# colinsongf/keyword_spotting

Measured on AMD Instinct MI355X. Metric: mel-frames/s (real-time 10 ms-hop audio streams sustained = value/100), higher is better.
Workload: dtype f32

## Files before the change

keyword_spotting_amd/csrc/gru_resident.hip:

```cpp
#include <cstddef>

#include "gru_device.h"
#include "launch.h"
#include "window_device.h"

namespace kws {

#if KWS_RESIDENT_VGPR_FORM
template <class... A> __device__ __forceinline__ void resident_prefence(A&...) {}
template <class... A> __device__ __forceinline__ void resident_fence(A&...) { __builtin_amdgcn_sched_barrier(0); }
#else
template <class... A> __device__ __forceinline__ void resident_prefence(A&... a) { mfma_prefence(a...); }
template <class... A> __device__ __forceinline__ void resident_fence(A&... a) { mfma_fence(a...); }
#endif


#if KWS_RESIDENT_VGPR_FORM
constexpr int resident_kreg(int kcx, bool first, bool last, bool window) { return first ? kcx : (last && window) ? 10 : 16; }
#else
constexpr int resident_kreg(int, bool first, bool, bool) { return first ? 0 : 2; }
#endif
constexpr size_t resident_lds_bytes(int kcx, bool first, bool last, bool window) {
    size_t n = 2 * 8 * 64 * 16 + (size_t)4 * (kcx - resident_kreg(kcx, first, last, window)) * 64 * 16;
    if (!first) n += 8 * 64 * 16;
    if (last) n += kPartialRingLdsBytes;
    if (first) n += (size_t)64 * xs_stride(kcx) * 4;
    return n;
}

template <int KCX, bool FIRST, bool LAST, bool MASKED, bool WINDOW>
__device__ __forceinline__ void gru_layer_resident_body(const GruLayerParams& p) {
    static_assert(!WINDOW || (LAST && !FIRST), "the window tail belongs to the last layer of a stack");
    static_assert(!WINDOW || !MASKED, "the window tail refuses seq_len");
    constexpr int H = 128, NT = 8, KCH = 32;
    const int tid = threadIdx.x;
    const int w = __builtin_amdgcn_readfirstlane(tid >> 6);
    const int lane = tid & 63, g = lane >> 4, s = lane & 15;
    const int n_groups = (p.B + kStreamsPerGroup - 1) / kStreamsPerGroup;
    int group = blockIdx.x;
    int b_raw = group * kStreamsPerGroup + s;
    bool bvalid = b_raw < p.B;
    int b = bvalid ? b_raw : p.B - 1;
    const int T = p.T;
    const int n0 = 2 * w, n1 = 2 * w + 1;

    extern __shared__ __attribute__((aligned(16))) char smem[];
    f32x4* hbuf = reinterpret_cast<f32x4*>(smem);
    f32x4* rhbuf = hbuf + NT * 64;
    constexpr int KREG = resident_kreg(KCX, FIRST, LAST, WINDOW), KL = KCX - KREG;
    static_assert(KREG >= 0 && KREG <= KCX && 192 + 4 * KREG <= 256, "the register chunks share the 256 AGPRs with the recurrent weights");
    f32x4* wlds = rhbuf + NT * 64;
    f32x4* xsb = wlds + 4 * KL * 64;
    char* const lds_tail = reinterpret_cast<char*>(xsb + (FIRST ? 0 : NT * 64));
    static_assert(resident_lds_bytes(KCX, FIRST, LAST, WINDOW) + (WINDOW ? kWinTailWordsBytes : 0) <= 160 * 1024, "LDS per CU");
    float* const pring = reinterpret_cast<float*>(lds_tail);
    int8_t* const cwords = WINDOW ? reinterpret_cast<int8_t*>(lds_tail + kPartialRingLdsBytes) : nullptr;
    const uint8_t* win_dl = reinterpret_cast<const uint8_t*>(cwords) + 16 * kWinTailWordsStride;
    constexpr size_t kWinOffset = offsetof(GruLayerParams, win);
    if constexpr (WINDOW) window_tail_prepare(window_tail_params_from_kernarg(kWinOffset), const_cast<uint8_t*>(win_dl), tid);
    constexpr int kXsStride = xs_stride(KCX);
    float* xs = reinterpret_cast<float*>(lds_tail + (LAST ? kPartialRingLdsBytes : 0));

    float wgh[2][2][KCH];
    float wch[2][KCH];
    float wcx[2][KCX];
    float wgx[KREG ? KREG : 1][4];
    const f32x4* wh4 = reinterpret_cast<const f32x4*>(p.wh);
#pragma unroll
    for (int j = 0; j < 2; ++j) {
        const int n = 2 * w + j;
#pragma unroll
        for (int k4 = 0; k4 < KCH / 4; ++k4) {
            const f32x4 vr = wh4[((n * 3 + 0) * (KCH / 4) + k4) * 64 + lane];
            const f32x4 vu = wh4[((n * 3 + 1) * (KCH / 4) + k4) * 64 + lane];
            const f32x4 vc = wh4[((n * 3 + 2) * (KCH / 4) + k4) * 64 + lane];
#pragma unroll
            for (int e = 0; e < 4; ++e) {
                wgh[j][0][4 * k4 + e] = vr[e];
                wgh[j][1][4 * k4 + e] = vu[e];
                wch[j][4 * k4 + e] = vc[e];
            }
        }
    }
    if constexpr (FIRST) {
#pragma unroll
        for (int j = 0; j < 2; ++j)
#pragma unroll
            for (int kc = 0; kc < KCX; ++kc) wcx[j][kc] = p.wx[(((2 * w + j) * 3 + 2) * KCX + kc) * 64 + lane];
#pragma unroll
        for (int kc = 0; kc < KCX; ++kc) {
            f32x4 v;
            v.x = p.wx[((n0 * 3 + 0) * KCX + kc) * 64 + lane];
            v.y = p.wx[((n0 * 3 + 1) * KCX + kc) * 64 + lane];
            v.z = p.wx[((n1 * 3 + 0) * KCX + kc) * 64 + lane];
            v.w = p.wx[((n1 * 3 + 1) * KCX + kc) * 64 + lane];
            if (kc < KREG) { const int kr = kc < KREG ? kc : 0; wgx[kr][0] = v[0]; wgx[kr][1] = v[1]; wgx[kr][2] = v[2]; wgx[kr][3] = v[3]; }
            else wlds[(w * KL + kc - KREG) * 64 + lane] = v;
        }
    } else {
        const f32x4* wx4 = reinterpret_cast<const f32x4*>(p.wx);
#pragma unroll
        for (int j = 0; j < 2; ++j)
#pragma unroll
            for (int k4 = 0; k4 < KCX / 4; ++k4) {
                const f32x4 vc = wx4[(((2 * w + j) * 3 + 2) * (KCX / 4) + k4) * 64 + lane];
#pragma unroll
                for (int e = 0; e < 4; ++e) wcx[j][4 * k4 + e] = vc[e];
            }
#pragma unroll
        for (int k4 = 0; k4 < KCX / 4; ++k4) {
            const f32x4 r0 = wx4[((n0 * 3 + 0) * (KCX / 4) + k4) * 64 + lane];
            const f32x4 u0 = wx4[((n0 * 3 + 1) * (KCX / 4) + k4) * 64 + lane];
            const f32x4 r1 = wx4[((n1 * 3 + 0) * (KCX / 4) + k4) * 64 + lane];
            const f32x4 u1 = wx4[((n1 * 3 + 1) * (KCX / 4) + k4) * 64 + lane];
#pragma unroll
            for (int e = 0; e < 4; ++e) {
                const f32x4 v = {r0[e], u0[e], r1[e], u1[e]};
                const int kc = 4 * k4 + e, kr = kc < KREG ? kc : 0;
                if (kc < KREG) { wgx[kr][0] = v[0]; wgx[kr][1] = v[1]; wgx[kr][2] = v[2]; wgx[kr][3] = v[3]; }
                else wlds[(w * KL + kc - KREG) * 64 + lane] = v;
            }
        }
    }
#pragma unroll
    for (int j = 0; j < 2; ++j) {
#pragma unroll
        for (int kc = 0; kc < KCH; ++kc) {
            asm volatile("" : "+a"(wgh[j][0][kc]));
            asm volatile("" : "+a"(wgh[j][1][kc]));
            asm volatile("" : "+a"(wch[j][kc]));
        }
    }
#if KWS_RESIDENT_VGPR_FORM
    if constexpr (KREG > 0) {
#pragma unroll
        for (int kc = 0; kc < KREG; ++kc)
#pragma unroll
            for (int e = 0; e < 4; ++e) asm volatile("" : "+a"(wgx[kc][e]));
    }
#endif
    asm volatile("s_nop 7" ::: "memory");
    f32x4 bias_r[2], bias_u[2], bias_c[2];
#pragma unroll
    for (int j = 0; j < 2; ++j) {
        const int n = 2 * w + j;
        bias_r[j] = ld4(p.bias + 0 * H + n * 16 + 4 * g);
        bias_u[j] = ld4(p.bias + 1 * H + n * 16 + 4 * g);
        bias_c[j] = ld4(p.bias + 2 * H + n * 16 + 4 * g);
    }
    float wfc[2][4];
    f32x4 bfc4 = splat4(0.f);
    if (LAST) {
#pragma unroll
        for (int j = 0; j < 2; ++j)
#pragma unroll
            for (int e = 0; e < 4; ++e) wfc[j][e] = p.wfc[((2 * w + j) * 4 + e) * 64 + lane];
        if (w == 0) bfc4 = ld4(p.bfc + 4 * g);
    }

    int len_s = T;
    int carry = -1;
    f32x4 hreg[2];
    const float4* xl_src = nullptr;
    const float4* xprev = nullptr;
    const float4* xg_next = nullptr;
    constexpr int XQ = KCX;
    const int xl_row = lane / XQ, xl_q = lane % XQ;
    const bool xl_active = FIRST && lane < 4 * XQ;
    auto enter_group = [&]() {
        b_raw = group * kStreamsPerGroup + s;
        bvalid = b_raw < p.B;
        b = bvalid ? b_raw : p.B - 1;
        const bool do_reset = p.reset != nullptr && p.reset[b] != 0;
        if constexpr (MASKED) len_s = p.seq_len ? p.seq_len[b] - p.t_base : T;
#pragma unroll
        for (int j = 0; j < 2; ++j) {
            const int n = 2 * w + j;
            hreg[j] = do_reset ? splat4(0.f) : ld4(p.state_in + (size_t)b * H + n * 16 + 4 * g);
            hbuf[n * 64 + lane] = hreg[j];
        }
        if (LAST) {
            carry = carried_word(p.prev_word, p.reset, group * kStreamsPerGroup + 4 * w + (lane >> 4), p.B);
        }
        if constexpr (FIRST) {
            const int xl_b = min(group * kStreamsPerGroup + 4 * w + (xl_active ? xl_row : 0), p.B - 1);
            xl_src = reinterpret_cast<const float4*>(p.x_mel + (size_t)xl_b * (p.t_stride ? p.t_stride : T) * p.I) + xl_q;
        } else {
            xprev = p.x_prev + (size_t)group * T * NT * 64 + lane;
            xg_next = xprev + ((size_t)(1 < T ? 1 : 0) * NT + n0) * 64;
        }
    };

    constexpr bool kIssueAtEnd = FIRST && !LAST;
    float4 xl_inflight = make_float4(0.f, 0.f, 0.f, 0.f);
    auto coop_issue = [&](int t_req) {
        const int t = t_req < T ? t_req : T - 1;
        if (xl_active) xl_inflight = xl_src[(size_t)t * XQ];
    };
    auto coop_commit = [&]() {
        if (xl_active) {
            float* dst = xs + (4 * (4 * w + xl_row)) * kXsStride + xl_q;
            dst[0 * kXsStride] = xl_inflight.x;
            dst[1 * kXsStride] = xl_inflight.y;
            dst[2 * kXsStride] = xl_inflight.z;
            dst[3 * kXsStride] = xl_inflight.w;
        }
    };
    float xbuf0[KCX];
    auto read_xs = [&](float (&dst)[KCX]) {
        const float* row = xs + (4 * s + g) * kXsStride;
#pragma unroll
        for (int k4 = 0; k4 < KCX / 4; ++k4) {
            const f32x4 v = *reinterpret_cast<const f32x4*>(row + 4 * k4);
            dst[4 * k4 + 0] = v[0]; dst[4 * k4 + 1] = v[1]; dst[4 * k4 + 2] = v[2]; dst[4 * k4 + 3] = v[3];
        }
        if constexpr (KCX % 4 >= 2) {
            const f32x2 v = *reinterpret_cast<const f32x2*>(row + (KCX / 4) * 4);
            dst[(KCX / 4) * 4 + 0] = v[0]; dst[(KCX / 4) * 4 + 1] = v[1];
        }
        if constexpr (KCX % 2 == 1) dst[KCX - 1] = row[KCX - 1];
    };
    auto load_x_slice = [&](float (&dst)[KCX], int t_req, const int sl) {
        if constexpr (!FIRST) {
            const int t = t_req < T ? t_req : T - 1;
            const float4 v = xprev[((size_t)t * NT + sl) * 64];
            dst[4 * sl + 0] = v.x; dst[4 * sl + 1] = v.y; dst[4 * sl + 2] = v.z; dst[4 * sl + 3] = v.w;
        }
    };
    float4 xg_inflight[2];
    auto group_issue = [&](int t_req) {
        if constexpr (!FIRST) {
            xg_inflight[0] = xg_next[0];
            xg_inflight[1] = xg_next[64];
            if (t_req + 1 < T) xg_next += NT * 64;
        }
    };
    auto group_commit = [&]() {
        if constexpr (!FIRST) {
#pragma unroll
            for (int j = 0; j < 2; ++j)
                xsb[(2 * w + j) * 64 + lane] = (f32x4){xg_inflight[j].x, xg_inflight[j].y, xg_inflight[j].z, xg_inflight[j].w};
        }
    };
    auto read_x_slice = [&](float (&dst)[KCX], const int sl) {
        if constexpr (!FIRST) {
            const f32x4 v = xsb[sl * 64 + lane];
            dst[4 * sl + 0] = v[0]; dst[4 * sl + 1] = v[1]; dst[4 * sl + 2] = v[2]; dst[4 * sl + 3] = v[3];
        }
    };

    f32x4 acc_r[2], acc_u[2], acc_c[2];
    auto gates_x_part = [&](const float (&xB)[KCX], auto k0_, auto k1_, auto pin_) {
        constexpr int K0 = decltype(k0_)::value, K1 = decltype(k1_)::value;
        constexpr bool PIN = decltype(pin_)::value;
        constexpr int R0 = K0 < KREG ? KREG : K0;
        f32x4 ring[3];
        if (R0 < K1) ring[R0 % 3] = wlds[(w * KL + R0 - KREG) * 64 + lane];
        if (R0 + 1 < K1) ring[(R0 + 1) % 3] = wlds[(w * KL + R0 + 1 - KREG) * 64 + lane];
#pragma unroll
        for (int kc = K0; kc < K1; ++kc) {
            if (kc + 2 < K1 && kc + 2 >= R0 + 2) ring[(kc + 2) % 3] = wlds[(w * KL + kc + 2 - KREG) * 64 + lane];
            if (PIN) __builtin_amdgcn_sched_barrier(0);
            const int kr = kc < KREG ? kc : 0;
            const f32x4 a4 = kc < KREG ? (f32x4){wgx[kr][0], wgx[kr][1], wgx[kr][2], wgx[kr][3]} : ring[kc % 3];
            acc_r[0] = mfma4(a4.x, xB[kc], acc_r[0]);
            acc_u[0] = mfma4(a4.y, xB[kc], acc_u[0]);
            acc_r[1] = mfma4(a4.z, xB[kc], acc_r[1]);
            acc_u[1] = mfma4(a4.w, xB[kc], acc_u[1]);
            if (PIN) __builtin_amdgcn_sched_barrier(0);
        }
    };
    using pinned = std::true_type;
    constexpr int KSPLIT = KCX / 2;
    using k_lo = std::integral_constant<int, 0>;
    using k_mid = std::integral_constant<int, KSPLIT>;
    using k_hi = std::integral_constant<int, KCX>;
    auto cand_x = [&](const float (&xB)[KCX]) {
#pragma unroll
        for (int j = 0; j < 2; ++j) acc_c[j] = bias_c[j];
#pragma unroll
        for (int kc = 0; kc < KCX; ++kc) {
            acc_c[0] = mfma4(wcx[0][kc], xB[kc], acc_c[0]);
            acc_c[1] = mfma4(wcx[1][kc], xB[kc], acc_c[1]);
        }
    };

    f32x4 hb_a, hb_b;

    auto frame = [&](int t, float (&xcur)[KCX], float (&xnxt)[KCX]) {
        resident_prefence(acc_r[0], acc_u[0], acc_r[1], acc_u[1]);
#pragma unroll
        for (int nn = 0; nn < NT; ++nn) {
            const f32x4 hb = (nn & 1) ? hb_b : hb_a;
            if (nn + 2 < NT) {
                if (nn & 1) hb_b = hbuf[(nn + 2) * 64 + lane]; else hb_a = hbuf[(nn + 2) * 64 + lane];
            }
            if constexpr (FIRST) { if (!kIssueAtEnd && nn == 0) coop_issue(t + 2); }
            else { if (nn == 0) group_issue(t + 2); read_x_slice(xnxt, nn); }
            __builtin_amdgcn_sched_barrier(0);
#pragma unroll
            for (int e = 0; e < 4; ++e) {
                const int kc = 4 * nn + e;
                const float hv = hb[e];
                KWS_MFMA_A(acc_r[0], wgh[0][0][kc], hv);
                KWS_MFMA_A(acc_u[0], wgh[0][1][kc], hv);
                KWS_MFMA_A(acc_r[1], wgh[1][0][kc], hv);
                KWS_MFMA_A(acc_u[1], wgh[1][1][kc], hv);
            }
        }
        resident_fence(acc_r[0], acc_u[0], acc_r[1], acc_u[1]);
        if constexpr (FIRST) read_xs(xcur);
        f32x4 u[2];
#pragma unroll
        for (int j = 0; j < 2; ++j) {
            const f32x2 r_lo = sigmoid2((f32x2){acc_r[j][0], acc_r[j][1]});
            const f32x2 r_hi = sigmoid2((f32x2){acc_r[j][2], acc_r[j][3]});
            const f32x2 rh_lo = r_lo * (f32x2){hreg[j][0], hreg[j][1]};
            const f32x2 rh_hi = r_hi * (f32x2){hreg[j][2], hreg[j][3]};
            rhbuf[(2 * w + j) * 64 + lane] = (f32x4){rh_lo.x, rh_lo.y, rh_hi.x, rh_hi.y};
        }
#pragma unroll
        for (int j = 0; j < 2; ++j) {
            const f32x2 u_lo = sigmoid2((f32x2){acc_u[j][0], acc_u[j][1]});
            const f32x2 u_hi = sigmoid2((f32x2){acc_u[j][2], acc_u[j][3]});
            u[j] = (f32x4){u_lo.x, u_lo.y, u_hi.x, u_hi.y};
        }
#pragma unroll
        for (int j = 0; j < 2; ++j) { acc_r[j] = bias_r[j]; acc_u[j] = bias_u[j]; }
        __builtin_amdgcn_sched_barrier(0);
        gates_x_part(xcur, k_lo{}, k_mid{}, pinned{});
        lds_barrier();
        hb_a = rhbuf[0 * 64 + lane];
        hb_b = rhbuf[1 * 64 + lane];
        group_commit();
        gates_x_part(xcur, k_mid{}, k_hi{}, pinned{});

        resident_prefence(acc_c[0], acc_c[1]);
#pragma unroll
        for (int nn = 0; nn < NT; ++nn) {
            const f32x4 rb = (nn & 1) ? hb_b : hb_a;
            if (nn + 2 < NT) {
                if (nn & 1) hb_b = rhbuf[(nn + 2) * 64 + lane]; else hb_a = rhbuf[(nn + 2) * 64 + lane];
            }
            __builtin_amdgcn_sched_barrier(0);
#pragma unroll
            for (int e = 0; e < 4; ++e) {
                const int kc = 4 * nn + e;
                const float rv = rb[e];
                KWS_MFMA_A(acc_c[0], wch[0][kc], rv);
                KWS_MFMA_A(acc_c[1], wch[1][kc], rv);
            }
        }
        resident_fence(acc_c[0], acc_c[1]);
        const unsigned live = !MASKED || t < len_s ? 0xffffffffu : 0u;
        f32x4 hout[2];
#pragma unroll
        for (int j = 0; j < 2; ++j) {
#pragma unroll
            for (int h2 = 0; h2 < 2; ++h2) {
                const f32x2 c = tanh2((f32x2){acc_c[j][2 * h2], acc_c[j][2 * h2 + 1]});
                const f32x2 uu = {u[j][2 * h2], u[j][2 * h2 + 1]};
                const f32x2 hh = {hreg[j][2 * h2], hreg[j][2 * h2 + 1]};
                const f32x2 hn = __builtin_elementwise_fma(uu, hh, (1.0f - uu) * c);
                if constexpr (!MASKED) {
                    hreg[j][2 * h2] = hn.x;
                    hreg[j][2 * h2 + 1] = hn.y;
                    continue;
                }
                hreg[j][2 * h2] = bitsel(live, hn.x, hh.x);
                hreg[j][2 * h2 + 1] = bitsel(live, hn.y, hh.y);
                if (LAST) {
                    hout[j][2 * h2] = bitsel(live, hn.x, 0.f);
                    hout[j][2 * h2 + 1] = bitsel(live, hn.y, 0.f);
                }
            }
        }
#pragma unroll
        for (int j = 0; j < 2; ++j) acc_c[j] = bias_c[j];
        constexpr int NCX = 2 * KCX;
        constexpr int NPOST = NCX >= 32 ? 16 : 8;
        constexpr int NPRE = NCX - NPOST;
        auto cand_x_mfma = [&](auto mc) {
            constexpr int m = decltype(mc)::value, kc = m / 2;
            if constexpr (m % 2 == 0) acc_c[0] = mfma4(wcx[0][kc], xcur[kc], acc_c[0]);
            else acc_c[1] = mfma4(wcx[1][kc], xcur[kc], acc_c[1]);
        };
        if constexpr (FIRST) {
            coop_commit();
            if constexpr (kIssueAtEnd) coop_issue(t + 3);
        }
#pragma unroll
        for (int j = 0; j < 2; ++j) {
            hbuf[(2 * w + j) * 64 + lane] = hreg[j];
            if (!LAST) {
                const f32x4 o = hreg[j];
                p.h_out[((size_t)group * T + t) * NT * 64 + (2 * w + j) * 64 + lane] =
                    make_float4(o[0], o[1], o[2], o[3]);
            }
        }
        if constexpr (LAST) {
            __builtin_amdgcn_sched_barrier(0);
            f32x4 accf = bfc4;
#pragma unroll
            for (int j = 0; j < 2; ++j)
#pragma unroll
                for (int e = 0; e < 4; ++e) accf = mfma4(wfc[j][e], MASKED ? hout[j][e] : hreg[j][e], accf);
            if (g < 2) *reinterpret_cast<f32x4*>(partial_slot(pring, t) + (w * 16 + s) * 8 + 4 * g) = accf;
        }
        __builtin_amdgcn_sched_barrier(0);
        static_for<0, NPRE>(cand_x_mfma);
        __builtin_amdgcn_sched_barrier(0);
        lds_barrier();
        hb_a = hbuf[0 * 64 + lane];
        hb_b = hbuf[1 * 64 + lane];
        __builtin_amdgcn_sched_barrier(0);
        static_for<NPRE, NCX>(cand_x_mfma);
        __builtin_amdgcn_sched_barrier(0);
        if constexpr (LAST) {
            if (((t + 1) & (kRingFrames - 1)) == 0 || t == T - 1) {
                const int t0 = t & ~(kRingFrames - 1);
                epilogue_flush_partials(p, pring, cwords, group, t0, t - t0 + 1, w, lane, t == T - 1, carry);
            }
        }
    };

    for (; group < n_groups; group += gridDim.x) {
    enter_group();
    if constexpr (!FIRST) {
        if (T > 0) {
            group_issue(1);
#pragma unroll
            for (int sl = 0; sl < NT; ++sl) load_x_slice(xbuf0, 0, sl);
            group_commit();
        }
    }
    __syncthreads();
    if (T > 0) {
        if constexpr (FIRST) {
            coop_issue(0);
            coop_commit();
            __syncthreads();
            read_xs(xbuf0);
            coop_issue(1);
        }
#pragma unroll
        for (int j = 0; j < 2; ++j) { acc_r[j] = bias_r[j]; acc_u[j] = bias_u[j]; }
        gates_x_part(xbuf0, k_lo{}, k_hi{}, pinned{});
        hb_a = hbuf[0 * 64 + lane];
        hb_b = hbuf[1 * 64 + lane];
        cand_x(xbuf0);
        if constexpr (FIRST) {
            __syncthreads();
            coop_commit();
            if constexpr (kIssueAtEnd) coop_issue(2);
            __syncthreads();
        }
    }
    for (int t = 0; t < T; ++t) frame(t, xbuf0, xbuf0);

    if (bvalid) {
#pragma unroll
        for (int j = 0; j < 2; ++j)
            *reinterpret_cast<f32x4*>(p.state_out + (size_t)b * H + (2 * w + j) * 16 + 4 * g) = hreg[j];
    }
    __syncthreads();
    if constexpr (WINDOW) {
        const WindowTail win = window_tail_params_from_kernarg(kWinOffset);
        WindowTailRegs<2> wreq;
        window_tail_request<2>(win, p.B, group * kStreamsPerGroup, tid, wreq);
        window_tail<2>(win, p.B, group * kStreamsPerGroup, T, cwords, kWinTailWordsStride, win_dl, reinterpret_cast<char*>(hbuf), tid, wreq);
        __syncthreads();
    }
    }
}

template <int KCX, bool FIRST, bool LAST, bool WINDOW = false>
__global__ void __launch_bounds__(256) __attribute__((amdgpu_waves_per_eu(1, 1)))
gru_layer_resident(const GruLayerParams p) { gru_layer_resident_body<KCX, FIRST, LAST, false, WINDOW>(p); }
template <int KCX, bool FIRST, bool LAST>
__global__ void __launch_bounds__(256) __attribute__((amdgpu_waves_per_eu(1, 1)))
gru_layer_resident_masked(const GruLayerParams p) { gru_layer_resident_body<KCX, FIRST, LAST, true, false>(p); }
template <int KCX, bool FIRST, bool LAST, bool MASKED>
inline constexpr auto resident_kernel = MASKED ? &gru_layer_resident_masked<KCX, FIRST, LAST> : &gru_layer_resident<KCX, FIRST, LAST, false>;

int gru_resident_kcx(int in_dim, bool first) { return first ? (in_dim + 3) / 4 : 32; }

bool gru_resident_supported(int hidden, int in_dim, bool first) {
    if (hidden != 128) return false;
    if (!first) return in_dim == 128;
    return in_dim == 32 || in_dim == 40 || in_dim == 48 || in_dim == 60 || in_dim == 64;
}

bool gru_resident_takes_window(bool first, bool last) { return last && !first; }

hipError_t launch_gru_layer_resident(const GruLayerParams& p, bool first, bool last, hipStream_t st) {
    const bool window = p.win.tab != nullptr;
    const size_t lds = resident_lds_bytes(p.KCX, first, last, window);
    const dim3 grid(persistent_grid(p.B));
    if (window) {
        if (!gru_resident_takes_window(first, last) || p.seq_len) return hipErrorInvalidValue;
        return launch_lds<gru_layer_resident<32, false, true, true>>(grid, dim3(256), lds + kWinTailWordsBytes, st, p);
    }
    return with_bool(p.seq_len != nullptr, [&](auto ma) {
        return with_bool(last, [&](auto la) {
            if (!first) return launch_lds<resident_kernel<32, false, la(), ma()>>(grid, dim3(256), lds, st, p);
            return with_int<8, 10, 12, 15, 16>(p.KCX, [&](auto kcx) {
                return launch_lds<resident_kernel<kcx(), true, la(), ma()>>(grid, dim3(256), lds, st, p);
            });
        });
    });
}

}
```

keyword_spotting_amd/csrc/kws_internal.h:

```cpp
#pragma once
#include <hip/hip_runtime.h>
#include <stdint.h>

#include "kws_amd.h"

#if defined(KWS_FAULT_INJECT) || defined(KWS_ABL_NOFLUSH) || defined(KWS_ABL_NOMEL) || defined(KWS_F16_TIMING) || defined(KWS_FE_TIMING) || \
    defined(KWS_FE_OCC) || defined(KWS_FE_FT) || defined(KWS_FE_SF) || defined(KWS_FE_NOSTAGE) || defined(KWS_FE_NODFT) || defined(KWS_FE_NOMEL) || \
    defined(KWS_OABL_NODIV) || defined(KWS_OABL_NODOT) || defined(KWS_OVERLAP_MIN_T) || defined(KWS_EXP_F16_WLO_ZERO)
#ifndef KWS_VARIANT_BUILD
#error "an experiment switch (KWS_FAULT_INJECT / KWS_ABL_* / KWS_*_TIMING / KWS_FE_* / KWS_OABL_* / KWS_OVERLAP_MIN_T) is defined in a product build: use tools/build_variant.sh"
#endif
#endif
#ifdef KWS_VARIANT_BUILD
#define KWS_VARIANT_TAG_1(name) "; " #name
#ifdef KWS_FAULT_INJECT
#define KWS_TAG_FAULT KWS_VARIANT_TAG_1(FAULT_INJECT)
#else
#define KWS_TAG_FAULT ""
#endif
#ifdef KWS_ABL_NOFLUSH
#define KWS_TAG_NOFLUSH KWS_VARIANT_TAG_1(ABL_NOFLUSH)
#else
#define KWS_TAG_NOFLUSH ""
#endif
#ifdef KWS_ABL_NOMEL
#define KWS_TAG_NOMEL KWS_VARIANT_TAG_1(ABL_NOMEL)
#else
#define KWS_TAG_NOMEL ""
#endif
#if defined(KWS_F16_TIMING) || defined(KWS_FE_TIMING)
#define KWS_TAG_TIMING KWS_VARIANT_TAG_1(TIMING)
#else
#define KWS_TAG_TIMING ""
#endif
#ifdef KWS_EXP_F16_WLO_ZERO
#define KWS_TAG_WLO KWS_VARIANT_TAG_1(EXP_F16_WLO_ZERO)
#else
#define KWS_TAG_WLO ""
#endif
#define KWS_VARIANT_TAG "; VARIANT BUILD" KWS_TAG_FAULT KWS_TAG_NOFLUSH KWS_TAG_NOMEL KWS_TAG_TIMING KWS_TAG_WLO
#else
#define KWS_VARIANT_TAG ""
#endif

namespace kws {

constexpr int kStreamsPerGroup = 16;
constexpr int kMaxClasses = 8;

struct WindowTail {
    uint8_t* tab;
    uint32_t* meta;
    int* head;
    int* count;
    const uint8_t* delta;
    const uint8_t* clear_before;
    int32_t* hit;
    uint8_t* restart;
    int nq, n_label;
};
constexpr int kWinTailMaxFrames = 64;
constexpr int kWinTailMaxChunks = 24;
constexpr int kWinTailWordsStride = kWinTailMaxFrames + 4;
constexpr size_t kWinTailWordsBytes = (size_t)16 * kWinTailWordsStride + 256;
__host__ __device__ inline size_t window_tail_scratch_bytes(int nq) { return (size_t)16 * (nq * 32 + 32); }

struct GruLayerParams {
    const float* wx;
    const float* wh;
    const float* bias;
    const float* wfc;
    const float* bfc;
    const float* x_mel;
    const float4* x_prev;
    float4* h_out;
    const float* state_in;
    float* state_out;
    const int32_t* seq_len;
    const uint8_t* reset;
    float* logits;
    float* softmax;
    int8_t* tokens;
    int32_t* prev_word;
    float decode_thres;
    float value_clip;
    int use_relu;
    int B, T, I, C;
    int t_stride;
    int t_base;
    int KCX;
    const int* ready_in;
    int* ready_out;
    int* pipe_error;
    WindowTail win;
};
struct GruStackParams {
    GruLayerParams layer[8];
    int L, G;
    int xcd_affine;
};
hipError_t launch_gru_stack_generic_pipelined(const GruStackParams& sp, int hidden, hipStream_t st);

struct GruWrapLayer {
    const float* igamma;
    float ibeta;
    int residual;
};
struct GruWrapParams { GruWrapLayer layer[8]; };
constexpr size_t gru_wrapped_extra_lds(int kx4) { return (size_t)kx4 * 64 * 16; }
hipError_t launch_gru_layer_generic_wrapped(const GruLayerParams& p, const GruWrapLayer& wl, int hidden, bool first, bool last,
                                            hipStream_t st);
hipError_t launch_gru_stack_generic_pipelined_wrapped(const GruStackParams& sp, const GruWrapParams& wp, int hidden, hipStream_t st);

struct GruBf16Params {
    const uint4* w[2];
    const float* bias[2];
    const uint4* wfc;
    const float* bfc;
    const float* x_mel;
    const float* state_in;
    float* state_out;
    const int32_t* seq_len;
    const uint8_t* reset;
    GruLayerParams epi;
    int B, T, I, L;
};
bool gru_bf16_supported(int hidden, int n_mel, int layers);
hipError_t launch_gru_stack_bf16(const GruBf16Params& p, int kx0, int nl, hipStream_t st);
bool gru_stack_bf16_takes_window(int kx0, int nl);
const char* gru_stack_bf16_kernel_name(int kx0, int nl);
bool gru_bf16_vgpr_form();

struct GruF16Params {
    const uint4* w;
    const float* bias;
    const uint4* wfc;
    const float* bfc;
    const float* x_mel;
    const uint4* x_prev;
    uint4* h_out;
    const float* state_in;
    float* state_out;
    const int32_t* seq_len;
    const uint8_t* reset;
    GruLayerParams epi;
    int B, T, I;
};
struct GruF16StackParams {
    GruF16Params layer[8];
    int L, G;
    int xcd_affine;
};
static_assert(sizeof(GruF16StackParams) <= 4096, "kernel arguments");
bool gru_f16x3_generic_supported(int hidden, int n_mel);
hipError_t launch_gru_layer_f16x3_generic(const GruF16Params& p, int hidden, bool first, bool last, hipStream_t st);
hipError_t launch_gru_stack_f16x3_pipelined(const GruF16StackParams& sp, int hidden, hipStream_t st);
bool gru_f16x3_supported(int hidden, int n_mel);
hipError_t launch_gru_layer_f16x3(const GruF16Params& p, bool first, bool last, hipStream_t st);
bool gru_f16x3_vgpr_form();

struct GruOctbitParams {
    const uint32_t* wg;
    const uint32_t* wc;
    const float* bias;
    const float* b127;
    float scale_g, scale_c;
    const float4* x_prev;
    float4* h_out;
    const float* state_in;
    float* state_out;
    const int32_t* seq_len;
    const uint8_t* reset;
    uint32_t* aq;
    float2* range;
    int B, T;
};
struct OctbitFcParams {
    const uint32_t* wfc;
    const float* b127;
    const float* bfc;
    float scale_w;
    const float4* h_top;
    float2* range;
    int range_ready;
    const int32_t* prev_in;
    float* logits; float* softmax; int8_t* tokens; int32_t* prev_word;
    float decode_thres, value_clip;
    int use_relu, B, T, C;
};
hipError_t launch_gru_layer_octbit(const GruOctbitParams& p, hipStream_t st);
hipError_t launch_octbit_fc(const OctbitFcParams& p, hipStream_t st);

struct DenseHead {
    const float* wfc;
    const float* bfc;
    float* logits;
    float* softmax;
    int8_t* tokens;
    int32_t* prev_word;
    const int32_t* prev_in;
    float decode_thres;
    int C;
};
struct DenseHeadsParams {
    const float4* h_top;
    const int32_t* seq_len;
    const uint8_t* reset;
    float* nn_outputs;
    DenseHead head[2];
    float value_clip;
    int use_relu, B, T;
};
constexpr int kHeadFrames = 32;
constexpr int kHeadsMaxFrames = 65535 * kHeadFrames;
hipError_t launch_dense_heads(const DenseHeadsParams& p, int hidden, hipStream_t st);

struct HeadsWindowHead {
    const float* wfc;
    const float* bfc;
    float* softmax;
    float decode_thres;
    int C;
};
struct HeadsWindowParams {
    const float4* h_top;
    HeadsWindowHead head[2];
    WindowTail win[2];
    int32_t* hit;
    uint8_t* restart;
    const int32_t* frames;
    const uint8_t* skip;
    float value_clip;
    int use_relu, B, T;
};
constexpr size_t kHeadsWindowLogitsBytes = (size_t)2 * 16 * kHeadFrames * 8 * sizeof(float);
__host__ __device__ inline int heads_window_stride(int T) { return T > 0 ? (T + 15) & ~15 : 16; }
__host__ __device__ inline size_t heads_window_lds_bytes(int T, int nq1, int nq2) {
    return kHeadsWindowLogitsBytes + (size_t)2 * 16 * heads_window_stride(T) + 512 + window_tail_scratch_bytes(nq1) + window_tail_scratch_bytes(nq2);
}
hipError_t launch_heads_window(const HeadsWindowParams& p, int hidden, hipStream_t st);

struct BankRef {
    const float* Wn;
    const float* bn;
    const int32_t* user;
    int capacity, n_new;
};
struct BankHeadsParams { DenseHeadsParams d; BankRef bank; };
struct BankWindowParams { HeadsWindowParams w; BankRef bank; };
struct BankSlotKeyword {
    uint8_t delta[256];
    int32_t n_label, n_used, own, pad;
};
static_assert(sizeof(BankSlotKeyword) == 272, "16-byte loads of the matcher");
struct BankKeywordHeadsParams { BankHeadsParams b; const BankSlotKeyword* slots; };
struct BankKeywordWindowParams { BankWindowParams b; const BankSlotKeyword* slots; };
constexpr size_t kBankHeadsLogitsBytes = (size_t)2 * 16 * (kHeadFrames + 1) * 8 * sizeof(float);
constexpr size_t kBankHeadsWordsBytes = (size_t)2 * 16 * (kHeadFrames + 1) * sizeof(int);
__host__ __device__ inline size_t bank_stage_bytes(int H, int n_new) { return ((size_t)16 * H * n_new + 128) * sizeof(float); }
__host__ __device__ inline size_t bank_heads_lds_bytes(int H, int n_new) { return kBankHeadsLogitsBytes + kBankHeadsWordsBytes + bank_stage_bytes(H, n_new); }
__host__ __device__ inline size_t bank_window_lds_bytes(int T, int nq1, int nq2, int H, int n_new) {
    return heads_window_lds_bytes(T, nq1, nq2) + bank_stage_bytes(H, n_new);
}
constexpr size_t kBankKeywordStageBytes = (size_t)16 * 256 + 16 * 2 * sizeof(int);
__host__ __device__ inline size_t bank_keyword_window_lds_bytes(int T, int nq1, int nq2, int H, int n_new) {
    return bank_window_lds_bytes(T, nq1, nq2, H, n_new) + kBankKeywordStageBytes;
}
hipError_t launch_bank_set_keyword(BankSlotKeyword* dst, const BankSlotKeyword& v, hipStream_t st);
hipError_t launch_bank_heads(const BankHeadsParams& p, const BankSlotKeyword* slots, int hidden, hipStream_t st);
hipError_t launch_bank_heads_window(const BankWindowParams& p, const BankSlotKeyword* slots, int hidden, hipStream_t st);

struct WindowParams {
    int8_t* words;
    int* lens;
    int* head;
    int* count;
    const float* softmax;
    const uint8_t* clear_before;
    int32_t* hit;
    uint8_t* restart;
    int32_t label[16];
    int label_len;
    float thres;
    int B, T, C, nq, tmax;
};
hipError_t launch_window_step(const WindowParams& p, hipStream_t st);
struct WindowIncParams {
    WindowTail win;
    uint8_t delta[256];
    const float* softmax;
    float thres;
    int B, T, C;
    const int32_t* frames;
    const uint8_t* skip;
};
hipError_t launch_window_inc(const WindowIncParams& p, hipStream_t st);
hipError_t launch_window_reset(int B, int* head, int* count, hipStream_t st);
hipError_t launch_window_reset_masked(const uint8_t* slots, int B, int* head, int* count, hipStream_t st);
struct StreamRecycleParams {
    const uint8_t* slots;
    float* state;
    uint8_t* restart;
    int *head, *count;
    const float* carry_in;
    float* carry_out;
    int32_t* len_out;
    int n_carry, carry_out_stride, L, B, H;
};
hipError_t launch_stream_recycle(const StreamRecycleParams& p, hipStream_t st);

struct FrontendParams {
    const float* pcm;
    const int16_t* pcm_i16;
    int gate;
    int fft_blocks;
    float vad_thres;
    const uint8_t* restart;
    uint8_t* silent;
    uint8_t* reset;
    float* next;
    int n_next;
    const float* carry;
    float* mel;
    const float* dft;
    const float* melw;
    int n_samples, T, fft, hop, n_mel, nf_tiles, mel_tiles, kc4, B, n_carry;
#ifdef KWS_FE_TIMING
    long long* timing;
#endif
    int mel_lo[4], mel_cnt[4], mel_off[4];
    const int32_t* lens;
    const int32_t* carry_len;
    int32_t* next_len;
    int32_t* frames;
    uint8_t* skip;
    int n_max, carry_stride;
    const float* dct;
    int n_mfcc, dct_tiles;
    int power;
    int centred;
    float pre_emphasis;
    const float* win;
};
hipError_t launch_mel_frontend(const FrontendParams& p, int B, hipStream_t st);
hipError_t launch_mel_fft400(const FrontendParams& p, int B, hipStream_t st);
hipError_t launch_features_fft400(const FrontendParams& p, int B, hipStream_t st);
hipError_t launch_linear_fft400(const FrontendParams& p, int B, int32_t* frames_out, float* energy_out, hipStream_t st);
constexpr int kPlanInts = 8;
struct PlanRow {
    int32_t src, noise, start, noise_avail, factor_bits, frames, pad[2];
};
static_assert(sizeof(PlanRow) == kPlanInts * sizeof(int32_t), "a plan row is kPlanInts ints");
struct AugmentRows {
    const int32_t *frames, *noise_frames;
    const float *energy, *noise_energy;
    const int32_t *src, *noise, *start;
    const float* gain_db;
    int B, K, R, T, Tn;
    int32_t* plan;
};
hipError_t launch_augment_fft400(const FrontendParams& p, const float* spec, const float* noise_spec, const AugmentRows& rows, hipStream_t st);
hipError_t launch_carry_tail(const float* carry, int n_carry, const float* chunk, int n_chunk, float* next, int n_next, int B,
                             hipStream_t st);

bool gru_resident_supported(int hidden, int in_dim, bool first);
int gru_resident_kcx(int in_dim, bool first);
hipError_t launch_gru_layer_resident(const GruLayerParams& p, bool first, bool last, hipStream_t st);
bool gru_resident_takes_window(bool first, bool last);
hipError_t launch_gru_layer_generic(const GruLayerParams& p, int hidden, bool first, bool last,
                                    hipStream_t st);

hipError_t launch_ctc_decode(int kind, const float* softmax, const int32_t* lengths, int B, int T, int C,
                             int lockout, float thres, float loose_thres, int32_t* words,
                             int32_t* counts, int max_words, hipStream_t st);
hipError_t launch_ctc_predict(const int32_t* words, const int32_t* counts, int B, int max_words,
                              const int32_t* label_digits, int label_len, int32_t* hit, hipStream_t st);
hipError_t launch_vad(const float* pcm, int B, int N, float thres, uint8_t* speech, float* abs_sum,
                      hipStream_t st);

hipError_t launch_state_passthrough(const float* state_in, float* state_out, const uint8_t* reset, int32_t* prev_word, int L, int B, int H,
                                    hipStream_t st);
hipError_t launch_vad_gate(const void* pcm, int pcm_int16, int B, int N, float thres, float* pcm_f32, const uint8_t* restart,
                           uint8_t* silent, uint8_t* reset, const float* carry, int n_carry, float* next, int n_next, hipStream_t st);

__host__ __device__ inline size_t ctc_wave_lds_floats(int T, int S_max) { return (size_t)T * (8 + 2 * S_max + 1); }
inline size_t ctc_loss_lds_bytes(int T, int S_max) { return sizeof(float) * ctc_wave_lds_floats(T, S_max); }
inline size_t enroll_fit_lds_bytes(int H, int n, int K, int T, int S_max) {
    return sizeof(float) * ((size_t)(3 + K) * (H + 1) * n + (size_t)K * ctc_wave_lds_floats(T, S_max));
}
hipError_t launch_ctc_loss(const float* logits, const int32_t* seq_len, const int32_t* labels, const int32_t* label_len, int B, int T, int C,
                           int S_max, float* loss, float* grad, hipStream_t st);
constexpr int kBeamMax = 32, kBeamRow = 64, kBeamCandidates = 8 * kBeamMax;
inline size_t ctc_beam_lds_bytes(int T) {
    return sizeof(float) * 8 * (size_t)T + kBeamCandidates * (8 + 4) + kBeamMax * 3 * 4 + 2 * kBeamMax * kBeamRow;
}
hipError_t launch_ctc_beam(const float* logits, const int32_t* seq_len, int B, int T, int C, int W, int K, int L_max, int merge_repeated,
                           int32_t* paths, int32_t* lengths, float* log_prob, hipStream_t st);
struct EnrollFitParams {
    const float *nn, *logits1;
    const int32_t *seq_len, *labels, *label_len;
    float *W, *b, *mW, *mb, *vW, *vb;
    float* loss_trace;
    float lr;
    int K, n, C, T, S_max, iterations, step0;
};
hipError_t launch_enroll_fit(const EnrollFitParams& p, int hidden, int E, hipStream_t st);

struct TrainForwardParams {
    const float* xg;
    const float* wh;
    const int32_t* seq_len;
    const uint8_t* drop;
    float *ar, *au, *ac, *hp, *rh;
    float* y;
    float keep_prob;
    int B, T;
};
struct TrainBackwardParams {
    const float* dy;
    const float* wht;
    const int32_t* seq_len;
    const uint8_t* drop;
    const float *ar, *au, *ac, *hp;
    float* dhat;
    float keep_prob;
    int B, T;
};
hipError_t launch_gru_train_forward(const TrainForwardParams& p, int hidden, hipStream_t st);
hipError_t launch_gru_train_backward(const TrainBackwardParams& p, int hidden, hipStream_t st);
struct TrainRowsGemm {
    const float* a; int lda;
    const uint8_t* live;
    const float* w; int swk, swn;
    const float* bias;
    float* out; int ldo;
    int M, K, N;
};
hipError_t launch_train_rows_gemm(const TrainRowsGemm& p, hipStream_t st);
enum { kWgradRows = 0, kWgradOnes = 1, kWgradInput = 2 };
struct TrainWgradJob {
    const float* a; const float* d;
    size_t out;
    int src, lda, K, ldd, N, ldo, unit0, pad;
};
hipError_t launch_train_wgrad(const TrainWgradJob* jobs, int njobs, int units, const float* x, const uint8_t* live, int M, int chunk_rows,
                              int chunks, float* partial, size_t P, hipStream_t st);
constexpr int kTrainReduceSpan = 1024;
inline int train_reduce_blocks(size_t P) { return (int)((P + kTrainReduceSpan - 1) / kTrainReduceSpan); }
hipError_t launch_train_reduce(const float* partial, int chunks, size_t P, float* grad, double* sumsq, hipStream_t st);
hipError_t launch_train_update(float* theta, float* m, float* v, const float* grad, const double* sumsq, int nblocks, size_t P, int adam,
                               float lr_t, float max_grad_norm, float* grad_norm_or_null, hipStream_t st);
struct TrainPackLayer { const float *wg, *bg, *wc, *bc; float *wx, *wh, *wht, *b3; int in; };
struct TrainPackParams { TrainPackLayer layer[8]; int L, H; };
hipError_t launch_train_pack(const TrainPackParams& p, hipStream_t st);
hipError_t launch_train_rowmask(const int32_t* seq_len, int B, int T, uint8_t* live, hipStream_t st);
hipError_t launch_train_scale(float* g, const float* logits, size_t rows, int C, float s, hipStream_t st);

hipError_t launch_octbit_matmul(const float* x, const int8_t* Wq, float scale_w, const float* bias,
                                float* out, int A, int K, int N, int per_row, float* range_ws,
                                hipStream_t st);

}
```

Measured before the change: 413.5 million.

## Reschedule first-layer input staging and update-gate sigmoid inside candidate h-loop

In the first GRU layer, the xs LDS read moves earlier, into the gate loop at nn=NT-2. The cooperative mel-frame commit and the next global issue are spread across the candidate h-part MFMA loop. The update-gate sigmoid is deferred until after the candidate MFMAs so its VALU work overlaps. Pad lanes now mirror real lanes and write into an extra LDS pad region, which removes divergence on the loads and stores. Experiment macros for the KSPLIT/NPOST knobs are added but stay off by default.

```diff
diff --git a/keyword_spotting_amd/csrc/gru_resident.hip b/keyword_spotting_amd/csrc/gru_resident.hip
--- a/keyword_spotting_amd/csrc/gru_resident.hip
+++ b/keyword_spotting_amd/csrc/gru_resident.hip
@@ -14,6 +14,9 @@
 template <class... A> __device__ __forceinline__ void resident_fence(A&... a) { mfma_fence(a...); }
 #endif
 
+
+constexpr int xs_pad_lanes(int kcx) { return 64 - 4 * kcx; }
+constexpr size_t xs_pad_floats(int kcx) { return xs_pad_lanes(kcx) > 0 ? (size_t)3 * xs_stride(kcx) + xs_pad_lanes(kcx) : 0; }
 
 #if KWS_RESIDENT_VGPR_FORM
 constexpr int resident_kreg(int kcx, bool first, bool last, bool window) { return first ? kcx : (last && window) ? 10 : 16; }
@@ -24,7 +27,7 @@
     size_t n = 2 * 8 * 64 * 16 + (size_t)4 * (kcx - resident_kreg(kcx, first, last, window)) * 64 * 16;
     if (!first) n += 8 * 64 * 16;
     if (last) n += kPartialRingLdsBytes;
-    if (first) n += (size_t)64 * xs_stride(kcx) * 4;
+    if (first) n += ((size_t)64 * xs_stride(kcx) + xs_pad_floats(kcx)) * 4;
     return n;
 }
 
@@ -165,8 +168,10 @@
     const float4* xprev = nullptr;
     const float4* xg_next = nullptr;
     constexpr int XQ = KCX;
-    const int xl_row = lane / XQ, xl_q = lane % XQ;
-    const bool xl_active = FIRST && lane < 4 * XQ;
+    const bool xl_real = lane < 4 * XQ;
+    const int xl_lane = xl_real ? lane : lane - 4 * XQ;
+    const int xl_row = xl_lane / XQ, xl_q = xl_lane % XQ;
+    static_assert(!FIRST || (64 - 4 * XQ >= 0 && 64 - 4 * XQ <= 4 * XQ), "every pad lane has a real lane to mirror");
     auto enter_group = [&]() {
         b_raw = group * kStreamsPerGroup + s;
         bvalid = b_raw < p.B;
@@ -183,7 +188,7 @@
             carry = carried_word(p.prev_word, p.reset, group * kStreamsPerGroup + 4 * w + (lane >> 4), p.B);
         }
         if constexpr (FIRST) {
-            const int xl_b = min(group * kStreamsPerGroup + 4 * w + (xl_active ? xl_row : 0), p.B - 1);
+            const int xl_b = min(group * kStreamsPerGroup + 4 * w + xl_row, p.B - 1);
             xl_src = reinterpret_cast<const float4*>(p.x_mel + (size_t)xl_b * (p.t_stride ? p.t_stride : T) * p.I) + xl_q;
         } else {
             xprev = p.x_prev + (size_t)group * T * NT * 64 + lane;
@@ -192,20 +197,18 @@
     };
 
     constexpr bool kIssueAtEnd = FIRST && !LAST;
+    constexpr bool kStageInCandH = kIssueAtEnd && 4 * KCX < 64;
     float4 xl_inflight = make_float4(0.f, 0.f, 0.f, 0.f);
     auto coop_issue = [&](int t_req) {
         const int t = t_req < T ? t_req : T - 1;
-        if (xl_active) xl_inflight = xl_src[(size_t)t * XQ];
-    };
-    auto coop_commit = [&]() {
-        if (xl_active) {
-            float* dst = xs + (4 * (4 * w + xl_row)) * kXsStride + xl_q;
-            dst[0 * kXsStride] = xl_inflight.x;
-            dst[1 * kXsStride] = xl_inflight.y;
-            dst[2 * kXsStride] = xl_inflight.z;
-            dst[3 * kXsStride] = xl_inflight.w;
-        }
-    };
+        xl_inflight = xl_src[(size_t)t * XQ];
+    };
+    auto coop_commit_half = [&](const int h) {
+        float* dst = xl_real ? xs + (4 * (4 * w + xl_row)) * kXsStride + xl_q : xs + 64 * kXsStride + (lane - 4 * XQ);
+        dst[(2 * h) * kXsStride] = h ? xl_inflight.z : xl_inflight.x;
+        dst[(2 * h + 1) * kXsStride] = h ? xl_inflight.w : xl_inflight.y;
+    };
+    auto coop_commit = [&]() { coop_commit_half(0); coop_commit_half(1); };
     float xbuf0[KCX];
     auto read_xs = [&](float (&dst)[KCX]) {
         const float* row = xs + (4 * s + g) * kXsStride;
@@ -271,7 +274,14 @@
         }
     };
     using pinned = std::true_type;
+#if defined(KWS_RESIDENT_KSPLIT)
+    constexpr int KSPLIT = FIRST ? (KWS_RESIDENT_KSPLIT < KCX ? KWS_RESIDENT_KSPLIT : KCX) : KCX / 2;
+#elif defined(KWS_RESIDENT_KSPLIT_UPPER)
+    constexpr int KSPLIT = FIRST ? KCX / 2 : KWS_RESIDENT_KSPLIT_UPPER;
+#else
     constexpr int KSPLIT = KCX / 2;
+#endif
+    static_assert(KSPLIT >= 0 && KSPLIT <= KCX, "the gate x-part split is a k-chunk index");
     using k_lo = std::integral_constant<int, 0>;
     using k_mid = std::integral_constant<int, KSPLIT>;
     using k_hi = std::integral_constant<int, KCX>;
@@ -295,7 +305,10 @@
             if (nn + 2 < NT) {
                 if (nn & 1) hb_b = hbuf[(nn + 2) * 64 + lane]; else hb_a = hbuf[(nn + 2) * 64 + lane];
             }
-            if constexpr (FIRST) { if (!kIssueAtEnd && nn == 0) coop_issue(t + 2); }
+            if constexpr (FIRST) {
+                if (!kIssueAtEnd && nn == 0) coop_issue(t + 2);
+                if (nn == NT - 2) read_xs(xcur);
+            }
             else { if (nn == 0) group_issue(t + 2); read_x_slice(xnxt, nn); }
             __builtin_amdgcn_sched_barrier(0);
 #pragma unroll
@@ -309,7 +322,6 @@
             }
         }
         resident_fence(acc_r[0], acc_u[0], acc_r[1], acc_u[1]);
-        if constexpr (FIRST) read_xs(xcur);
         f32x4 u[2];
 #pragma unroll
         for (int j = 0; j < 2; ++j) {
@@ -319,8 +331,10 @@
             const f32x2 rh_hi = r_hi * (f32x2){hreg[j][2], hreg[j][3]};
             rhbuf[(2 * w + j) * 64 + lane] = (f32x4){rh_lo.x, rh_lo.y, rh_hi.x, rh_hi.y};
         }
+        constexpr bool kUpdateGateInB = FIRST && 4 * KCX < 64;
 #pragma unroll
         for (int j = 0; j < 2; ++j) {
+            if constexpr (kUpdateGateInB) { u[j] = acc_u[j]; continue; }
             const f32x2 u_lo = sigmoid2((f32x2){acc_u[j][0], acc_u[j][1]});
             const f32x2 u_hi = sigmoid2((f32x2){acc_u[j][2], acc_u[j][3]});
             u[j] = (f32x4){u_lo.x, u_lo.y, u_hi.x, u_hi.y};
@@ -342,6 +356,11 @@
             if (nn + 2 < NT) {
                 if (nn & 1) hb_b = rhbuf[(nn + 2) * 64 + lane]; else hb_a = rhbuf[(nn + 2) * 64 + lane];
             }
+            if constexpr (kStageInCandH) {
+                if (nn == 2) coop_commit_half(0);
+                if (nn == 3) coop_commit_half(1);
+                if (nn == 4) coop_issue(t + 3);
+            }
             __builtin_amdgcn_sched_barrier(0);
 #pragma unroll
             for (int e = 0; e < 4; ++e) {
@@ -352,6 +371,15 @@
             }
         }
         resident_fence(acc_c[0], acc_c[1]);
+        if constexpr (kUpdateGateInB) {
+#pragma unroll
+            for (int j = 0; j < 2; ++j) {
+                asm volatile("" : "+v"(u[j]));
+                const f32x2 u_lo = sigmoid2((f32x2){u[j][0], u[j][1]});
+                const f32x2 u_hi = sigmoid2((f32x2){u[j][2], u[j][3]});
+                u[j] = (f32x4){u_lo.x, u_lo.y, u_hi.x, u_hi.y};
+            }
+        }
         const unsigned live = !MASKED || t < len_s ? 0xffffffffu : 0u;
         f32x4 hout[2];
 #pragma unroll
@@ -378,14 +406,18 @@
 #pragma unroll
         for (int j = 0; j < 2; ++j) acc_c[j] = bias_c[j];
         constexpr int NCX = 2 * KCX;
+#ifdef KWS_RESIDENT_NPOST
+        constexpr int NPOST = NCX >= 32 ? 16 : (KWS_RESIDENT_NPOST < NCX ? KWS_RESIDENT_NPOST : NCX);
+#else
         constexpr int NPOST = NCX >= 32 ? 16 : 8;
+#endif
         constexpr int NPRE = NCX - NPOST;
         auto cand_x_mfma = [&](auto mc) {
             constexpr int m = decltype(mc)::value, kc = m / 2;
             if constexpr (m % 2 == 0) acc_c[0] = mfma4(wcx[0][kc], xcur[kc], acc_c[0]);
             else acc_c[1] = mfma4(wcx[1][kc], xcur[kc], acc_c[1]);
         };
-        if constexpr (FIRST) {
+        if constexpr (FIRST && !kStageInCandH) {
             coop_commit();
             if constexpr (kIssueAtEnd) coop_issue(t + 3);
         }
diff --git a/keyword_spotting_amd/csrc/kws_internal.h b/keyword_spotting_amd/csrc/kws_internal.h
--- a/keyword_spotting_amd/csrc/kws_internal.h
+++ b/keyword_spotting_amd/csrc/kws_internal.h
@@ -6,9 +6,10 @@
 
 #if defined(KWS_FAULT_INJECT) || defined(KWS_ABL_NOFLUSH) || defined(KWS_ABL_NOMEL) || defined(KWS_F16_TIMING) || defined(KWS_FE_TIMING) || \
     defined(KWS_FE_OCC) || defined(KWS_FE_FT) || defined(KWS_FE_SF) || defined(KWS_FE_NOSTAGE) || defined(KWS_FE_NODFT) || defined(KWS_FE_NOMEL) || \
-    defined(KWS_OABL_NODIV) || defined(KWS_OABL_NODOT) || defined(KWS_OVERLAP_MIN_T) || defined(KWS_EXP_F16_WLO_ZERO)
+    defined(KWS_OABL_NODIV) || defined(KWS_OABL_NODOT) || defined(KWS_OVERLAP_MIN_T) || defined(KWS_EXP_F16_WLO_ZERO) || \
+    defined(KWS_RESIDENT_NPOST) || defined(KWS_RESIDENT_KSPLIT) || defined(KWS_RESIDENT_KSPLIT_UPPER)
 #ifndef KWS_VARIANT_BUILD
-#error "an experiment switch (KWS_FAULT_INJECT / KWS_ABL_* / KWS_*_TIMING / KWS_FE_* / KWS_OABL_* / KWS_OVERLAP_MIN_T) is defined in a product build: use tools/build_variant.sh"
+#error "an experiment switch (KWS_FAULT_INJECT / KWS_ABL_* / KWS_*_TIMING / KWS_FE_* / KWS_OABL_* / KWS_OVERLAP_MIN_T / KWS_RESIDENT_*) is defined in a product build: use tools/build_variant.sh"
 #endif
 #endif
 #ifdef KWS_VARIANT_BUILD
```

Result: no change. 417.2 million (median of 6 runs) (+0.9%).
